# michaelfeil/skyjo_rl

Measured on AMD Instinct MI355X. Metric: env-steps/sec (whole node) at 65 536 parallel 3-player games, higher is better.
Workload: dtype int8

## Files before the change

skyjo_rl_amd/csrc/skyjo_record.h:

```cpp
#pragma once
#ifndef SKYJO_DEVICE_PARTS
#error "include skyjo_device.h"
#endif

template <bool INDIRECT>
__device__ __forceinline__ void emit_record(const SkParams &P, uint8_t *lp, const HdrRegs &h, const ObsRegs &ob, int action,
                                            uint8_t *out, uint4 *held = nullptr, const uint4 *pre_a = nullptr, uint32_t pre_b = 0) {
  const int phase = h.w0 & 0xff;
  const uint32_t q0 = ob.q0, q1 = ob.q1, q2 = ob.q2;
  const uint32_t act24 = ((uint32_t)action & 0xffu) << 24;
  uint32_t m[8];
  {
    const uint32_t pm = phase ? 0xffffffffu : 0u;
    m[0] = ob.nz0 & pm, m[1] = ob.nz1 & pm, m[2] = ob.nz2 & pm, m[3] = ob.hd0 & pm, m[4] = ob.hd1 & pm, m[5] = ob.hd2 & pm;
    m[6] = (phase ? 0u : 0x0101u) | (((h.w0 >> 8) & 0xffu) << 16) | ((uint32_t)phase << 24);
    m[7] = (((h.w0 >> 16) & F_DONE) ? 1u : 0u) | ((h.w0 >> 24) << 8) | ((h.w2 & 0xffffu) << 16);
  }
  const uint4 a = pre_a ? *pre_a : LQ(1);
  const uint32_t s8 = (pre_a ? pre_b : (uint32_t)LB(32)) | ((h.w1 >> 24) << 8) | ((h.w2 >> 24) << 16);
  if (INDIRECT) {
    uint4 *o = (uint4 *)out;
    uint4 b;
    b.x = s8 | (q0 << 24), b.y = (q0 >> 8) | (q1 << 24), b.z = (q1 >> 8) | (q2 << 24), b.w = (q2 >> 8) | act24;
    if (held) {
      held[0] = a, held[1] = b, held[2] = make_uint4(m[0], m[1], m[2], m[3]), held[3] = make_uint4(m[4], m[5], m[6], m[7]);
    } else {
      o[0] = a, o[1] = b;
      o[2] = make_uint4(m[0], m[1], m[2], m[3]);
      o[3] = make_uint4(m[4], m[5], m[6], m[7]);
    }
  } else {
    uint32_t *o = (uint32_t *)out;
    const int N = P.L.N;
    o[0] = a.x, o[1] = a.y, o[2] = a.z, o[3] = a.w;
    uint32_t carry = s8;
    for (int p = 0; p < N; p++) {
      const uint4 r = LQ((sk_pb(P.L, p) + PB_VIS) >> 4);
      o[4 + 3 * p] = carry | (r.x << 24);
      o[5 + 3 * p] = (r.x >> 8) | (r.y << 24);
      o[6 + 3 * p] = (r.y >> 8) | (r.z << 24);
      carry = r.z >> 8;
    }
    o[4 + 3 * N] = carry | act24;
    uint32_t *om = o + (P.L.Dp >> 2);
#pragma unroll
    for (int w = 0; w < 8; w++) om[w] = m[w];
  }
}

__device__ __forceinline__ size_t bank_rec16(const SkParams &P, int slot, int g) {
  return ((size_t)slot * P.tiles * SK_TILE + (size_t)g) * P.L.chunks;
}
__device__ __forceinline__ void load_spare(const SkParams &P, uint8_t *lp, int slot, int tile, int lane) {
  const uint4 *s = P.spare + bank_rec16(P, slot, tile * SK_TILE + lane);
  const int n = P.L.chunks;
  for (int c = 0; c < n; c += 6) {
    uint4 v[6];
#pragma unroll
    for (int k = 0; k < 6; k++)
      if (c + k < n) v[k] = s[c + k];
#pragma unroll
    for (int k = 0; k < 6; k++)
      if (c + k < n) LQ(c + k) = v[k];
  }
}
__device__ __forceinline__ void store_spare(const SkParams &P, uint8_t *lp, int slot, int g) {
  uint4 *d = P.spare + bank_rec16(P, slot, g);
  const int n = P.L.chunks;
  for (int c = 0; c < n; c += 6) {
    uint4 v[6];
#pragma unroll
    for (int k = 0; k < 6; k++)
      if (c + k < n) v[k] = LQ(c + k);
#pragma unroll
    for (int k = 0; k < 6; k++)
      if (c + k < n) d[c + k] = v[k];
  }
}

__device__ __forceinline__ void bank_advance(const SkParams &P, uint8_t *lp, int g, int head, uint32_t dc) {
  const uint8_t nh = (uint8_t)((head + 1) % SK_BANK);
  P.bank_head[g] = nh;
  LB(H_BANK) = nh;
  P.deals_consumed[g] = dc + 1;
  P.done[g] = 0;
}

__device__ __forceinline__ bool consume_spare(const SkParams &P, uint8_t *lp, int tile, int lane, int g, int head) {
  const size_t G = (size_t)P.tiles * SK_TILE;
  const uint8_t ready = P.spare_ready[(size_t)head * G + g];
  const uint32_t dc = P.deals_consumed[g];
  if (!ready) return false;
  load_spare(P, lp, head, tile, lane);
  P.spare_ready[(size_t)head * G + g] = 0;
  bank_advance(P, lp, g, head, dc);
  return true;
}

struct SpareRegs {
  uint32_t dc;
  int head;
  uint8_t ready;
};
__device__ __forceinline__ void spare_issue(const SkParams &P, uint8_t *lp, uint32_t lds_tile, int tile, int lane, int g, SpareRegs &r) {
  const size_t G = (size_t)P.tiles * SK_TILE;
  r.head = LB(H_BANK) % SK_BANK;
  r.ready = P.spare_ready[(size_t)r.head * G + g];
  r.dc = P.deals_consumed[g];
  const uint32_t voff = (uint32_t)(bank_rec16(P, r.head, g) * 16);
  asm volatile("s_waitcnt lgkmcnt(0)" ::: "memory");
  dma_bank_record<false>((const uint8_t *)P.spare, voff, lds_tile, P.L.chunks);
}
__device__ __forceinline__ bool spare_commit(const SkParams &P, uint8_t *lp, int g, const SpareRegs &r) {
  sk_vm_drain();
  if (!r.ready) return false;
  P.spare_ready[(size_t)r.head * (size_t)P.tiles * SK_TILE + g] = 0;
  bank_advance(P, lp, g, r.head, r.dc);
  return true;
}

__device__ __forceinline__ constexpr int sk_stage_stride(int rec_bytes) { return ((rec_bytes >> 2) & 7) == 0 ? rec_bytes + 16 : rec_bytes; }

__device__ __forceinline__ bool deal_inline(const SkParams &P, uint8_t *lp, uint8_t *fp, int g, int tile, int lane, int head);
```

skyjo_rl_amd/csrc/skyjo_step.h:

```cpp
#pragma once
#ifndef SKYJO_DEVICE_PARTS
#error "include skyjo_device.h"
#endif

__device__ __forceinline__ void sk_publish_deals(const SkParams &P, int g) {
  const size_t G = (size_t)P.tiles * SK_TILE;
  const int b = P.busy[g];
  if (b) {
    const uint32_t tag = P.plan_tag[g];
    const uint32_t f = __hip_atomic_load(&P.done_flag[g], __ATOMIC_RELAXED, __HIP_MEMORY_SCOPE_AGENT);
    if ((f & 0x7fffffffu) == tag) {
      SK_FENCE_ACQUIRE(P);
      if (!P.cancel[g] && f == tag) P.spare_ready[(size_t)(b - 1) * G + g] = 1;
      P.busy[g] = 0, P.cancel[g] = 0;
    }
  }
}
__device__ __forceinline__ void sk_plan_deals(const SkParams &P, int g, int lane) {
  const size_t G = (size_t)P.tiles * SK_TILE;
  bool need = false, empty = false;
  if (g < P.B) {
    const uint8_t busy = P.busy[g];
    const int head = P.bank_head[g] % SK_BANK;
    const uint32_t consumed = P.deals_consumed[g];
    uint8_t ready[SK_BANK];
#pragma unroll
    for (int k = 0; k < SK_BANK; k++) ready[k] = P.spare_ready[(size_t)k * G + g];
    bool open = true;
    int r = 0;
#pragma unroll
    for (int k = 0; k < SK_BANK; k++) {
      uint8_t f = 0;
#pragma unroll
      for (int j = 0; j < SK_BANK; j++) f = (head + k) % SK_BANK == j ? ready[j] : f;
      open = open && f != 0;
      r += open ? 1 : 0;
    }
    need = !busy && r < SK_BANK;
    empty = need && r == 0;
    if (need) {
      P.busy[g] = (uint8_t)(1 + (head + r) % SK_BANK);
      P.cancel[g] = 0;
      P.plan_ep[g] = consumed + (uint32_t)r;
      P.plan_tag[g] = P.plan_new_tag;
    }
  }
  const unsigned long long be = __ballot(empty);
  if (be && lane == 0) atomicAdd(P.bank_empty + (P.be_add & 1u), (uint32_t)__popcll(be));
}

__device__ __forceinline__ void sk_error_to_host(const SkParams &P, int lane) {
  if (lane == 0) {
    const uint32_t e = __hip_atomic_load(P.dev_error, __ATOMIC_RELAXED, __HIP_MEMORY_SCOPE_AGENT);
    if (e) P.health_host[2] = e;
  }
}
__device__ __forceinline__ void sk_export_raw(const SkParams &P, uint8_t *lp, int g, uint8_t *o) {
  for (int c = 0; c < P.L.chunks; c++) ((uint4 *)o)[c] = LQ(c);
  double *d = (double *)(o + P.L.state_bytes);
  for (int p = 0; p < P.L.N; p++) d[p] = P.rewards[(size_t)g * P.L.N + p], d[P.L.N + p] = P.scores[(size_t)g * P.L.N + p];
  uint32_t *m = (uint32_t *)(d + 2 * P.L.N);
  m[0] = P.rng_mode == SKYJO_RNG_MT19937 ? (uint32_t)P.mt_idx[g] : 0u;
  m[1] = P.done[g];
}

__device__ __forceinline__ uint32_t sk_next_tag(uint32_t t) {
  t = (t + 1u) & 0x7fffffffu;
  return t ? t : 1u;
}
template <bool INDIRECT, bool POLICY, int NP, bool PLANAR = false>
__device__ __forceinline__ void step_body(const SkParams &Pin, const int tile, const int lane, uint32_t *lds_raw, const int32_t *actions,
                                          uint8_t *rec_out, int32_t *act_out, int iters, uint64_t policy_seed, uint64_t iter0,
                                          double *end_rew_out, uint8_t *end_out, uint8_t *raw_out, int raw_stride, const int cycle_len = 0,
                                          const bool defer_ok = true) {
  SkParams P = Pin;
  TRACE_DECL;
  if (NP > 0) P.L = sk_make_layout(NP, INDIRECT ? 1 : 0);
  const int g = tile * SK_TILE + lane;
  const uint32_t lds_tile = (uint32_t)(uintptr_t)(__attribute__((address_space(3))) uint32_t *)lds_raw;
  uint8_t *lp = (uint8_t *)lds_raw + lane * 16;
  uint8_t *stg = (uint8_t *)lds_raw + P.L.chunks * 1024;
  uint8_t *fp = stg + lane * 4;
  const int stg_bytes = (INDIRECT || PLANAR) ? 4096 : SK_TILE * (P.L.rec_bytes + 16);
  uint8_t *ap = stg + stg_bytes + lane * 8;
  constexpr bool DEFER = POLICY && NP > 0 && NP < 8;
  constexpr bool REGACC = NP > 0 && NP < 8;
  constexpr int NACC = REGACC ? SK_ACC_KINDS * NP : 1;
  double racc_store[NACC];
#pragma unroll
  for (int k = 0; k < NACC; k++) racc_store[k] = 0.0;
  double *racc = REGACC ? racc_store : nullptr;
  uint8_t *pendp = DEFER && defer_ok ? stg + stg_bytes + (REGACC ? 0 : SK_ACC_KINDS * P.L.N * 512) + lane * 16 : nullptr;
  int pend_fin = -1;
  if (!REGACC)
    for (int k = 0; k < SK_ACC_KINDS * P.L.N; k++) ACC(k) = 0.0;
  STAMP_DECL;
  if (!POLICY) tile_load(P, P.state, tile, lane, lp);
  else dma_record<true>((const uint8_t *)P.state, (uint32_t)((((size_t)tile * P.L.chunks) * SK_TILE + lane) * 16), lds_tile, P.L.chunks);
  if (P.ov_flags & 1u) sk_publish_deals(P, g);
  sk_vm_drain();
  HdrRegs h;
  HDR_LOAD(h);
  STAMP(0);
  const bool valid = ((h.w0 >> 16) & F_VALID) != 0;
  LaneCounters cnt;
  uint32_t r0 = 0, r1 = 0, r2 = 0, r3 = 0;
  const uint64_t gid = P.game_id0 + (uint64_t)g;
  ObsRegs ob;
  if (valid) obs_load(P, lp, (h.w0 >> 8) & 0xff, ob);
  for (int it = 0; it < iters; it++) {
    const uint64_t iter = iter0 + (uint64_t)it;
    if (POLICY && (it == 0 || (iter & 3) == 0)) {
      philox4x32_10((uint32_t)(iter >> 2), (uint32_t)gid, (uint32_t)(gid >> 32), 0x504F4C00u, (uint32_t)policy_seed,
                    (uint32_t)(policy_seed >> 32), r0, r1, r2, r3);
      for (int k = (int)(iter & 3); k > 0; k--) {
        const uint32_t t = r0;
        r0 = r1, r1 = r2, r2 = r3, r3 = t;
      }
    }
    STAMP_T(3);
    const uint32_t word = r0;
    if (POLICY) {
      r0 = r1, r1 = r2, r2 = r3, r3 = word;
    }
    int a = -1;
    if (valid) {
      const bool over = ((h.w0 >> 16) & F_DONE) != 0;
      if (!POLICY) a = actions[g];
      const bool skip = !POLICY && a == SKYJO_ACTION_SKIP;
      const bool acted = !over && !skip;
      SpareRegs sp;
      const bool resetting = over && P.auto_reset && !skip;
      if (resetting) spare_issue(P, lp, lds_tile, tile, lane, g, sp);
      STAMP_T(4);
      if (!over && !skip) {
        const uint32_t v0 = ob.q0, v1 = ob.q1, v2 = ob.q2;
        STAMP_N(2);
        const uint4 row_pre = LQ(sk_pb(P.L, (h.w0 >> 8) & 0xff) >> 4);
        asm volatile("" ::: "memory");
        if (POLICY) a = policy_pick(h.w0 & 0xff, ob, word);
#ifndef SK_STAMPS_FINE
        STAMP_N(3);
#endif
        apply_action<INDIRECT, NP, POLICY>(P, lp, fp, ap, h, v0, v1, v2, a, g, cnt, st, pendp, pend_fin, row_pre, racc);
#ifdef SK_STAMPS_FINE
        STAMP(6);
#else
        STAMP(5);
#endif
      } else if (!skip) {
        a = -1;
        if (P.auto_reset) {
          bool dealt = true;
          if (!spare_commit(P, lp, g, sp)) {
            dealt = deal_inline(P, lp, fp, g, tile, lane, sp.head);
            cnt.waits++;
          }
          HDR_LOAD(h);
          if (SK_OFTEN(dealt)) {
            h.w0 = (h.w0 & 0x00ffffffu) | ((uint32_t)SKYJO_ST_RESET << 24);
            cnt.resets++;
          }
        } else {
          h.w0 = (h.w0 & 0x00ffffffu) | ((uint32_t)SKYJO_ST_NOOP_DONE << 24);
        }
        STAMP(1);
      } else {
        a = -1;
      }
      if (!POLICY && acted && (unsigned)a >= (unsigned)SKYJO_NUM_ACTIONS) a = -2;
      if (!POLICY && end_out) {
        const bool end = acted && ((h.w0 >> 16) & F_DONE) != 0;
        end_out[g] = end ? 1 : 0;
        for (int q = 0; q < P.L.N; q++) end_rew_out[(size_t)g * P.L.N + q] = end ? P.rewards[(size_t)g * P.L.N + q] : 0.0;
      }
      const uint4 rec_a = LQ(1);
      const uint32_t rec_b = LB(32);
      const uint4 rec_row = LQ((sk_pb(P.L, (h.w0 >> 8) & 0xff) + PB_VIS) >> 4);
      asm volatile("" ::: "memory");
      obs_from_row(rec_row, ob);
      if (rec_out) {
        if (INDIRECT) {
          uint4 rr[4];
          emit_record<INDIRECT>(P, lp, h, ob, a, nullptr, rr, &rec_a, rec_b);
          if (PLANAR) {
            typedef uint32_t u32x4_t __attribute__((ext_vector_type(4)));
            uint8_t *blk = rec_out + ((size_t)it * P.tiles + (size_t)tile) * (SK_TILE * 64) + lane * 16;
#pragma unroll
            for (int p = 0; p < 4; p++) __builtin_nontemporal_store((u32x4_t){rr[p].x, rr[p].y, rr[p].z, rr[p].w}, (u32x4_t *)(blk + p * 1024));
          } else {
#pragma unroll
            for (int p = 0; p < 4; p++) *(uint4 *)(stg + lane * 64 + ((p + (lane >> 1)) & 3) * 16) = rr[p];
          }
        } else if (PLANAR) {
          constexpr int PIECES = NP > 0 ? (((19 + 12 * NP + 3) & ~3) + 32 + 15) / 16 : 1;
          uint32_t wbuf[4 * PIECES];
#pragma unroll
          for (int k = 0; k < 4 * PIECES; k++) wbuf[k] = 0u;
          emit_record<INDIRECT>(P, lp, h, ob, a, (uint8_t *)wbuf, nullptr, &rec_a, rec_b);
          typedef uint32_t u32x4_t __attribute__((ext_vector_type(4)));
          uint8_t *blk = rec_out + ((size_t)it * P.tiles + (size_t)tile) * (SK_TILE * 16 * PIECES) + lane * 16;
#pragma unroll
          for (int p = 0; p < PIECES; p++)
            __builtin_nontemporal_store((u32x4_t){wbuf[4 * p], wbuf[4 * p + 1], wbuf[4 * p + 2], wbuf[4 * p + 3]}, (u32x4_t *)(blk + p * 1024));
        } else {
          emit_record<INDIRECT>(P, lp, h, ob, a, stg + lane * sk_stage_stride(P.L.rec_bytes), nullptr, &rec_a, rec_b);
        }
      }
      if (act_out) __builtin_nontemporal_store(a, &act_out[(size_t)it * P.B + g]);
#ifdef SK_STAMPS_FINE
      STAMP(7);
#else
      STAMP(6);
#endif
    }
    if (DEFER && ((it & (SK_SCORE_EVERY - 1)) == SK_SCORE_EVERY - 1 || it == iters - 1)) {
      if (SK_RARE(__any(pend_fin >= 0))) {
        if (pend_fin >= 0) {
          finish_game_fixed<(NP > 0 && NP < 8) ? NP : 1>(P, pendp, 1024, ap, g, pend_fin, racc);
          pend_fin = -1;
        }
      }
    }
    if (!INDIRECT && !PLANAR && rec_out) {
      typedef uint32_t u32x4_t __attribute__((ext_vector_type(4)));
      const int pieces = P.L.rec_bytes >> 4, stride = sk_stage_stride(P.L.rec_bytes);
      uint8_t *blk = rec_out + ((size_t)it * P.B + (size_t)tile * SK_TILE) * (size_t)P.L.rec_bytes;
      const int live = P.B - tile * SK_TILE;
      for (int q0 = lane; q0 < pieces * SK_TILE; q0 += 4 * SK_TILE) {
        uint4 v[4];
#pragma unroll
        for (int j = 0; j < 4; j++) {
          const int q = q0 + j * SK_TILE, r = q / pieces, p = q - r * pieces;
          if (q < pieces * SK_TILE) v[j] = *(const uint4 *)(stg + r * stride + p * 16);
        }
        if (SK_OFTEN(live >= SK_TILE)) {
#pragma unroll
          for (int j = 0; j < 4; j++) {
            const int q = q0 + j * SK_TILE;
            if (q0 - lane + j * SK_TILE < pieces * SK_TILE)
              __builtin_nontemporal_store((u32x4_t){v[j].x, v[j].y, v[j].z, v[j].w}, (u32x4_t *)(blk + (size_t)q * 16));
          }
        } else {
#pragma unroll
          for (int j = 0; j < 4; j++) {
            const int q = q0 + j * SK_TILE, r = q / pieces;
            if (q < pieces * SK_TILE && r < live)
              __builtin_nontemporal_store((u32x4_t){v[j].x, v[j].y, v[j].z, v[j].w}, (u32x4_t *)(blk + (size_t)q * 16));
          }
        }
      }
    }
    if (INDIRECT && !PLANAR && rec_out) {
      typedef uint32_t u32x4_t __attribute__((ext_vector_type(4)));
      uint8_t *blk = rec_out + ((size_t)it * P.B + (size_t)tile * SK_TILE) * 64;
      const int live = P.B - tile * SK_TILE;
      uint4 v[4];
#pragma unroll
      for (int j = 0; j < 4; j++) {
        const int r = 16 * j + (lane >> 2), p = lane & 3;
        v[j] = *(const uint4 *)(stg + r * 64 + ((p + (r >> 1)) & 3) * 16);
      }
      if (SK_OFTEN(live >= SK_TILE)) {
#pragma unroll
        for (int j = 0; j < 4; j++)
          __builtin_nontemporal_store((u32x4_t){v[j].x, v[j].y, v[j].z, v[j].w}, (u32x4_t *)(blk + j * 1024 + lane * 16));
      } else {
#pragma unroll
        for (int j = 0; j < 4; j++)
          if (16 * j + (lane >> 2) < live)
            __builtin_nontemporal_store((u32x4_t){v[j].x, v[j].y, v[j].z, v[j].w}, (u32x4_t *)(blk + j * 1024 + lane * 16));
      }
    }
    STAMP_T(2);
    if (POLICY && cycle_len && it + 1 < iters && (it + 1) % cycle_len == 0) {
      if (P.busy[g]) (void)wait_deal_done(P, g);
      sk_publish_deals(P, g);
      sk_plan_deals(P, g, lane);
      P.plan_new_tag = sk_next_tag(P.plan_new_tag);
      TRACE_WAIT_BEGIN;
      __syncthreads();
      TRACE_WAIT_END;
    }
  }
  HDR_FLUSH(h);
  tile_store_nt(P, P.state, tile, lane, lp);
  if (!POLICY && raw_out && valid) sk_export_raw(P, lp, g, raw_out + (size_t)g * raw_stride);
  if (P.ov_flags & 2u) {
    if (P.ov_flags & 1u) {
      if (P.busy[g]) (void)wait_deal_done(P, g);
      sk_publish_deals(P, g);
    }
    sk_plan_deals(P, g, lane);
  }
  if (!POLICY) {
    sk_error_to_host(P, lane);
    if (P.host_seq) {
      __threadfence_system();
      if (lane == 0) __hip_atomic_store(&P.health_host[3], P.host_seq, __ATOMIC_RELEASE, __HIP_MEMORY_SCOPE_SYSTEM);
    }
  }
  uint32_t v[7] = {cnt.steps, cnt.episodes, cnt.illegal, cnt.resets, cnt.sum_len, cnt.reshuffles, cnt.waits};
#pragma unroll
  for (int k = 0; k < 7; k++)
    for (int off = 32; off > 0; off >>= 1) v[k] += __shfl_down(v[k], off, 64);
  if (lane == 0) {
    unsigned long long *c = P.tile_counters + (size_t)tile * 8;
#pragma unroll
    for (int k = 0; k < 7; k++) c[k] += v[k];
  }
  if (__any(cnt.episodes | cnt.illegal)) {
    double mine = 0.0;
    if (REGACC) {
#pragma unroll
      for (int k = 0; k < NACC; k++) {
        double x = racc_store[k];
        for (int off = 32; off > 0; off >>= 1) x += __shfl_down(x, off, 64);
        x = __shfl(x, 0, 64);
        mine = lane == k ? x : mine;
      }
    } else {
      for (int k = 0; k < SK_ACC_KINDS * P.L.N; k++) {
        double x = ACC(k);
        for (int off = 32; off > 0; off >>= 1) x += __shfl_down(x, off, 64);
        x = __shfl(x, 0, 64);
        mine = lane == k ? x : mine;
      }
    }
    if (lane < SK_ACC_KINDS * P.L.N)
      P.acc_tile[(size_t)tile * SK_ACC_KINDS * SKYJO_MAX_PLAYERS + (lane / P.L.N) * SKYJO_MAX_PLAYERS + lane % P.L.N] += mine;
  }
  STAMP(7);
  STAMP_STORE;
  TRACE_STORE(0, (uint32_t)(iter0 / (uint64_t)(iters > 0 ? iters : 1)), lane, tile);
}

template <bool INDIRECT, bool POLICY, int NP, bool PLANAR = false>
__global__ __launch_bounds__(SK_TILE) void k_step(SkParams Pin, const int32_t *actions, uint8_t *rec_out,
                                                  int32_t *act_out, int iters, uint64_t policy_seed, uint64_t iter0,
                                                  double *end_rew_out, uint8_t *end_out, uint8_t *raw_out, int raw_stride) {
  extern __shared__ uint32_t lds_raw[];
  step_body<INDIRECT, POLICY, NP, PLANAR>(Pin, (int)blockIdx.x, (int)threadIdx.x, lds_raw, actions, rec_out, act_out, iters, policy_seed, iter0,
                                          end_rew_out, end_out, raw_out, raw_stride);
}

template <bool INDIRECT>
__device__ __forceinline__ void sk_emit_to(const SkParams &P, uint8_t *lp, const HdrRegs &h, const ObsRegs &ob, uint8_t *rec_out, int tile, int lane,
                                           int planar) {
  const int g = tile * SK_TILE + lane;
  if (INDIRECT && planar) {
    uint4 rr[4];
    emit_record<INDIRECT>(P, lp, h, ob, -1, nullptr, rr);
    uint4 *o = (uint4 *)(rec_out + (size_t)tile * SK_TILE * P.L.rec_bytes) + lane;
#pragma unroll
    for (int k = 0; k < 4; k++) o[k * SK_TILE] = rr[k];
  } else {
    emit_record<INDIRECT>(P, lp, h, ob, -1, rec_out + (size_t)g * P.L.rec_bytes);
  }
}

template <bool INDIRECT>
__global__ __launch_bounds__(SK_TILE) void k_observe(SkParams P, const int32_t *players, uint8_t *rec_out, int planar) {
  extern __shared__ uint32_t lds_raw[];
  const int tile = blockIdx.x, lane = threadIdx.x, g = tile * SK_TILE + lane;
  uint8_t *lp = (uint8_t *)lds_raw + lane * 16;
  sk_error_to_host(P, lane);
  tile_load(P, P.state, tile, lane, lp);
  if (!(LB(H_FLAGS) & F_VALID)) return;
  HdrRegs h;
  HDR_LOAD(h);
  int q = players ? players[g] : LB(H_PLAYER);
  q = q < 0 ? 0 : (q >= P.L.N ? P.L.N - 1 : q);
  ObsRegs ob;
  obs_load(P, lp, q, ob);
  sk_emit_to<INDIRECT>(P, lp, h, ob, rec_out, tile, lane, planar);
}

template <bool INDIRECT>
__global__ __launch_bounds__(SK_TILE) void k_reset(SkParams P, const uint8_t *mask, uint8_t *rec_out, uint8_t *raw_out, int raw_stride, int planar) {
  extern __shared__ uint32_t lds_raw[];
  const int tile = blockIdx.x, lane = threadIdx.x, g = tile * SK_TILE + lane;
  uint8_t *lp = (uint8_t *)lds_raw + lane * 16;
  uint8_t *fp = (uint8_t *)lds_raw + P.L.chunks * 1024 + lane * 4;
  if (g >= P.B) return;
  const bool want = !mask || mask[g];
  bool want_counted = false;
  tile_load(P, P.state, tile, lane, lp);
  if (want) {
    const int head = P.bank_head[g] % SK_BANK;
    bool dealt = true;
    if (!consume_spare(P, lp, tile, lane, g, head)) dealt = deal_inline(P, lp, fp, g, tile, lane, head);
    if (dealt) LB(H_STATUS) = SKYJO_ST_RESET;
    want_counted = dealt;
  }
  HdrRegs h;
  HDR_LOAD(h);
  if (rec_out) {
    ObsRegs ob;
    obs_load(P, lp, LB(H_PLAYER), ob);
    sk_emit_to<INDIRECT>(P, lp, h, ob, rec_out, tile, lane, planar);
  }
  if (want) tile_store(P, P.state, tile, lane, lp);
  if (raw_out && (LB(H_FLAGS) & F_VALID)) sk_export_raw(P, lp, g, raw_out + (size_t)g * raw_stride);
  sk_error_to_host(P, lane);
  const unsigned long long wb = __ballot(want_counted);
  if (want_counted && lane == __ffsll((long long)wb) - 1) P.tile_counters[(size_t)tile * 8 + 3] += __popcll(wb);
}
```

Baseline: 48.17 billion.

## Cooperatively load spare deal records for resetting games across wavefront lanes

For 3-4 player policy runs, resetting games no longer each issue a per-lane DMA of the spare deal record into LDS. Up to three resetting games in a wavefront are served by the whole wave: lanes are split into three groups by exec masks, each lane loads one 16-byte chunk with a global_load_dwordx4, and a masked ds_write_b128 places it into the right LDS slot at commit. Any further resetting lanes fall back to the old DMA path. The aim is a wide coalesced load that replaces serialized per-lane record copies, at the cost of hand-written exec-mask assembly, extra reserved vector registers and a vmcnt(0) wait at commit.

New measurement: 49.45 billion, median of 6. +2.7%, better.

```diff
diff --git a/skyjo_rl_amd/csrc/skyjo_record.h b/skyjo_rl_amd/csrc/skyjo_record.h
--- a/skyjo_rl_amd/csrc/skyjo_record.h
+++ b/skyjo_rl_amd/csrc/skyjo_record.h
@@ -119,6 +119,78 @@
   return true;
 }
 
+typedef uint32_t sk_u32x4 __attribute__((ext_vector_type(4)));
+struct CoopRegs {
+  sk_u32x4 d;
+  uint32_t a, t;
+};
+__device__ __forceinline__ void sk_coop_reserve(CoopRegs &c) { asm volatile("; coop reserve %0 %1 %2" : "=v"(c.d), "=v"(c.a), "=v"(c.t)); }
+__device__ __forceinline__ void sk_coop_release(const CoopRegs &c) { asm volatile("; coop release %0 %1" ::"v"(c.d), "v"(c.a)); }
+__device__ __forceinline__ constexpr long long sk_lanes_lo(int a, int b) {
+  return (long long)(((b >= 64 ? ~0ull : (1ull << b) - 1ull) & ~((1ull << a) - 1ull)) & 0xffffffffull);
+}
+__device__ __forceinline__ constexpr long long sk_lanes_hi(int a, int b) {
+  return (long long)(((b >= 64 ? ~0ull : (1ull << b) - 1ull) & ~((1ull << a) - 1ull)) >> 32);
+}
+#define SK_COOP_E0 "s_mov_b32 exec_lo, %[e0l]\n\ts_mov_b32 exec_hi, %[e0h]\n\t"
+#define SK_COOP_E1 "s_mov_b32 exec_lo, %[e1l]\n\ts_mov_b32 exec_hi, %[e1h]\n\t"
+#define SK_COOP_E2 "s_mov_b32 exec_lo, %[e2l]\n\ts_mov_b32 exec_hi, %[e2h]\n\t"
+#define SK_COOP_MASKS(CH)                                                                                                   \
+  [ch] "n"(CH), [e0l] "n"(sk_lanes_lo(0, 3 * CH)), [e0h] "n"(sk_lanes_hi(0, 3 * CH)), [e1l] "n"(sk_lanes_lo(CH, 3 * CH)),   \
+      [e1h] "n"(sk_lanes_hi(CH, 3 * CH)), [e2l] "n"(sk_lanes_lo(2 * CH, 3 * CH)), [e2h] "n"(sk_lanes_hi(2 * CH, 3 * CH))
+template <int CH>
+__device__ __forceinline__ void spare_issue_coop(const SkParams &P, uint8_t *lp, uint32_t lds_tile, int lane, int g, SpareRegs &r, CoopRegs &c) {
+  static_assert(64 / CH == 3, "three or four players: three games per group");
+  const size_t G = (size_t)P.tiles * SK_TILE;
+  r.head = LB(H_BANK) % SK_BANK;
+  r.ready = P.spare_ready[(size_t)r.head * G + g];
+  r.dc = P.deals_consumed[g];
+  const uint32_t voff = (uint32_t)(bank_rec16(P, r.head, g) * 16);
+  unsigned long long m = __builtin_amdgcn_ballot_w64(true);
+  const int l0 = __ffsll((long long)m) - 1;
+  m &= m - 1;
+  const int l1 = m ? __ffsll((long long)m) - 1 : l0;
+  m &= m - 1;
+  const int l2 = m ? __ffsll((long long)m) - 1 : l0;
+  m &= m - 1;
+  const uint32_t s0 = __builtin_amdgcn_readlane(voff, l0), s1 = __builtin_amdgcn_readlane(voff, l1), s2 = __builtin_amdgcn_readlane(voff, l2);
+  const uint32_t a0 = lds_tile + 16u * (uint32_t)l0, a1 = 16u * (uint32_t)(l1 - l0), a2 = 16u * (uint32_t)(l2 - l1);
+  unsigned long long sv;
+  asm volatile("; coop request %[d] %[a] %[t]\n\ts_mov_b64 %[sv], exec\n\t" SK_COOP_E0
+               "v_mbcnt_lo_u32_b32 %[t], -1, 0\n\tv_mbcnt_hi_u32_b32 %[t], -1, %[t]\n\tv_mov_b32 %[a], %[s0]\n\t"
+               SK_COOP_E1 "v_mov_b32 %[a], %[s1]\n\tv_subrev_u32 %[t], %[ch], %[t]\n\t"
+               SK_COOP_E2 "v_mov_b32 %[a], %[s2]\n\tv_subrev_u32 %[t], %[ch], %[t]\n\t"
+               SK_COOP_E0 "v_lshl_add_u32 %[a], %[t], 4, %[a]\n\tglobal_load_dwordx4 %[d], %[a], %[base]\n\t"
+               "s_nop 0\n\tv_lshl_add_u32 %[a], %[t], 10, %[a0]\n\t"
+               SK_COOP_E1 "v_add_u32 %[a], %[a1], %[a]\n\t"
+               SK_COOP_E2 "v_add_u32 %[a], %[a2], %[a]\n\t"
+               "s_mov_b64 exec, %[sv]"
+               : [d] "+v"(c.d), [t] "+v"(c.t), [a] "+v"(c.a), [sv] "=&s"(sv)
+               : [base] "s"(P.spare), [s0] "s"(s0), [s1] "s"(s1), [s2] "s"(s2), [a0] "s"(a0), [a1] "s"(a1), [a2] "s"(a2), SK_COOP_MASKS(CH)
+               : "memory");
+  if (SK_RARE(m != 0)) {
+    if ((m >> lane) & 1) {
+      asm volatile("s_waitcnt lgkmcnt(0)" ::: "memory");
+      dma_bank_record<false>((const uint8_t *)P.spare, voff, lds_tile, CH);
+    }
+#ifdef SK_DIAG
+    if (lane == l0) P.stamps[(size_t)(g / SK_TILE) * 8 + 7] += (unsigned long long)__popcll(m);
+#endif
+  }
+}
+template <int CH>
+__device__ __forceinline__ bool spare_commit_coop(const SkParams &P, uint8_t *lp, int g, const SpareRegs &r, const CoopRegs &c) {
+  unsigned long long sv;
+  asm volatile("; coop commit %[d] %[a]\n\ts_waitcnt vmcnt(0)\n\ts_mov_b64 %[sv], exec\n\t" SK_COOP_E0 "ds_write_b128 %[a], %[d]\n\ts_waitcnt lgkmcnt(0)\n\ts_mov_b64 exec, %[sv]"
+               : [sv] "=&s"(sv)
+               : [a] "v"(c.a), [d] "v"(c.d), SK_COOP_MASKS(CH)
+               : "memory");
+  if (!r.ready) return false;
+  P.spare_ready[(size_t)r.head * (size_t)P.tiles * SK_TILE + g] = 0;
+  bank_advance(P, lp, g, r.head, r.dc);
+  return true;
+}
+
 __device__ __forceinline__ constexpr int sk_stage_stride(int rec_bytes) { return ((rec_bytes >> 2) & 7) == 0 ? rec_bytes + 16 : rec_bytes; }
 
 __device__ __forceinline__ bool deal_inline(const SkParams &P, uint8_t *lp, uint8_t *fp, int g, int tile, int lane, int head);
diff --git a/skyjo_rl_amd/csrc/skyjo_step.h b/skyjo_rl_amd/csrc/skyjo_step.h
--- a/skyjo_rl_amd/csrc/skyjo_step.h
+++ b/skyjo_rl_amd/csrc/skyjo_step.h
@@ -84,6 +84,9 @@
   const int stg_bytes = (INDIRECT || PLANAR) ? 4096 : SK_TILE * (P.L.rec_bytes + 16);
   uint8_t *ap = stg + stg_bytes + lane * 8;
   constexpr bool DEFER = POLICY && NP > 0 && NP < 8;
+  constexpr bool COOP = POLICY && NP >= 3 && NP <= 4;
+  constexpr int COOP_CH = COOP ? (H_PILE + SK_NCARDS + 15) / 16 + 2 * NP : 18;
+  static_assert(PB_BYTES == 32, "COOP_CH: two chunks per player");
   constexpr bool REGACC = NP > 0 && NP < 8;
   constexpr int NACC = REGACC ? SK_ACC_KINDS * NP : 1;
   double racc_store[NACC];
@@ -124,6 +127,8 @@
       r0 = r1, r1 = r2, r2 = r3, r3 = word;
     }
     int a = -1;
+    CoopRegs coop;
+    if (COOP) sk_coop_reserve(coop);
     if (valid) {
       const bool over = ((h.w0 >> 16) & F_DONE) != 0;
       if (!POLICY) a = actions[g];
@@ -131,7 +136,10 @@
       const bool acted = !over && !skip;
       SpareRegs sp;
       const bool resetting = over && P.auto_reset && !skip;
-      if (resetting) spare_issue(P, lp, lds_tile, tile, lane, g, sp);
+      if (resetting) {
+        if (COOP) spare_issue_coop<COOP_CH>(P, lp, lds_tile, lane, g, sp, coop);
+        else spare_issue(P, lp, lds_tile, tile, lane, g, sp);
+      }
       STAMP_T(4);
       if (!over && !skip) {
         const uint32_t v0 = ob.q0, v1 = ob.q1, v2 = ob.q2;
@@ -152,7 +160,7 @@
         a = -1;
         if (P.auto_reset) {
           bool dealt = true;
-          if (!spare_commit(P, lp, g, sp)) {
+          if (!(COOP ? spare_commit_coop<COOP_CH>(P, lp, g, sp, coop) : spare_commit(P, lp, g, sp))) {
             dealt = deal_inline(P, lp, fp, g, tile, lane, sp.head);
             cnt.waits++;
           }
@@ -214,6 +222,7 @@
       STAMP(6);
 #endif
     }
+    if (COOP) sk_coop_release(coop);
     if (DEFER && ((it & (SK_SCORE_EVERY - 1)) == SK_SCORE_EVERY - 1 || it == iters - 1)) {
       if (SK_RARE(__any(pend_fin >= 0))) {
         if (pend_fin >= 0) {
```
